# Mamba413/bess

Measured on AMD Instinct MI355X. Metric: candidate subsets solved/sec (n=50k,p=10k,k<=200 LM), higher is better.
Workload: dtype f64; 1 GPU; configs[1]: LM sequential path, Gaussian X n=50000 p=10000, s.list=1..200, GIC, warm start, max_iter=20, is_normal; score_pass=covariance updates (cached Gram columns), collective=none, ranks_with_work=1

## Files before the change

bess_amd/capi.py:

```python
import ctypes
import os
import sys

import numpy as np

_HERE = os.path.dirname(os.path.abspath(__file__))
LIB_PATH = os.environ.get("BESSX_LIB_PATH") or os.path.join(_HERE, "libbessx.so")

_D = ctypes.POINTER(ctypes.c_double)
_I = ctypes.POINTER(ctypes.c_int)
_i = ctypes.c_int
_d = ctypes.c_double
_ll = ctypes.c_longlong
_vp = ctypes.c_void_p

SYMBOLS = [
    "bessx_last_error", "bessx_device_info", "bessx_pywrap_bess", "bessx_bessCpp", "bessx_session_create",
    "bessx_session_destroy", "bessx_session_set_cv", "bessx_session_get_cv_folds", "bessx_session_sequential_path", "bessx_session_gs_path",
    "bessx_session_pgs_path", "bessx_session_get_screening", "bessx_session_get_screening_groups", "bessx_session_get_screening_scores", "bessx_session_score_mode", "bessx_session_counter",
    "bessx_session_trace_enable", "bessx_session_trace_size", "bessx_session_trace_copy_int",
    "bessx_session_trace_copy_double", "bessx_session_get_normalization", "bessx_session_score_pass_stats",
    "bessx_session_enable_kernel_timing", "bessx_session_submodel_steps", "bessx_session_fit", "bessx_session_fit_width", "bessx_session_reset_caches",
    "bessx_session_sequential_path_chain", "bessx_session_cv_eval", "bessx_session_debug_block_stream",
    "bessx_session_set_fill_hook", "bessx_session_set_kpath_chains",
# ... 575 lines not shown
        return int(lib().bessx_session_score_mode(self._h))

    def counters(self):
        names = {0: "chained_fits", 1: "cg_fallbacks", 2: "passes_over_X", 3: "chained_queued", 7: "cv_side_by_side_rounds",
                 8: "cv_union_fills", 9: "tie_rescues", 10: "cache_restarts", 11: "cv_contexts_dropped",
                 12: "cv_fold_contexts", 13: "shared_wide_fills", 14: "kpath_chunked_paths", 15: "kpath_stitch_refits",
                 16: "kpath_chunk_fills", 17: "kpath_chains_last_path",
                 18: "kpath_stitch_giveups", 19: "group_XTX_ns",
                 22: "kpath_coarse_us",
                 23: "kpath_chunks_us", 24: "kpath_stitch_us", 25: "panel_launches_one_group",
                 26: "panel_ns_one_group", 27: "panel_launches_two_groups", 28: "panel_ns_two_groups",
                 29: "shared_pass_launches", 30: "shared_pass_chain_slots", 31: "shared_pass_partial_batches",
                 32: "own_queue_streams_created_by_the_process", 33: "multi_responses_batched",
                 34: "multi_responses_host", 35: "multi_union_fills", 36: "x_bytes_uploaded_from_host",
                 37: "x_bytes_ingested_on_device", 38: "live_device_bytes_of_the_process",
                 39: "live_pinned_bytes_of_the_process", 40: "allocation_requests_of_the_process"}
        return {n: int(lib().bessx_session_counter(self._h, i)) for i, n in names.items()}

    def screening(self):
        a = np.zeros(self.p_kept, dtype=np.int32)
        lib().bessx_session_get_screening(self._h, _ip(a), a.size)
        return a

    def screening_groups(self):
        n = lib().bessx_session_get_screening_groups(self._h, None, 0)
        a = np.zeros(max(n, 1), dtype=np.int32)
        lib().bessx_session_get_screening_groups(self._h, _ip(a), n)
        return a[:n]

    def screening_scores(self):
        n = lib().bessx_session_get_screening_scores(self._h, None, 0)
# ... 1890 lines not shown
```

bess_amd/csrc/bessx_dev.h:

```cpp
#ifndef BESSX_DEV_H
#define BESSX_DEV_H

#include <hip/hip_runtime.h>

namespace bessx {

struct FitCtrl {
  int done;
  int l;
  int T0;
  int k_cur;
  int irls_done;
  int irls_steps;
  int info;
  int same_prev;
  double coef0;
  double ll0;
  int d_fresh;
  int irls_last;
  int fast_same;
  int ls_m;
  double ll1;
  int gram_full;
  int cov_nfill;
// ... 282 lines not shown
  int nblk, m;
  double *bcur, *bprev;
};
hipError_t launch_chol(const double *Gt, int m, int mt, double ridge, int ridge_skip0, const double *rhs,
                       const int *rhs_gather, double *sol, int *info, const FitCtrl *ctrl, int slot, int gate_mode,
                       hipStream_t st, const CholFuse *fuse = nullptr, const IrlsChk *chk = nullptr);
hipError_t launch_sym_fallback(const double *Gt, int m, int mt, double ridge, int ridge_skip0, const double *rhs,
                               const int *rhs_gather, double *sol, int *info, const FitCtrl *ctrl, int slot,
                               hipStream_t st, const CholFuse *fuse);
hipError_t launch_cg(int m, int mt, double ridge, const double *rhs, const int *A_new, double *sol, const FitCtrl *ctrl,
                     int slot, const CholFuse *fuse, int maxit, hipStream_t st, double tol = 1e-13, bool by_rows = true);
bool sel_cgr_applies(int len, int m);
hipError_t launch_sel_cgr(const double *score, int len, int k, int *A_new, const FitCtrl *ctrl, int slot,
                          const TopkNeed *need, double ridge, const double *rhs, double *sol, const CholFuse *fuse,
                          int maxit, hipStream_t st, double tol);
struct McState {
  int cand;
  int ncand;
  int need_d;
  int finished;
  int parked;
  int resume;
  int prev_fresh;
  int prev_T0;
  int solves;
  int why;
  int pad_[6];
};
static_assert(sizeof(McState) == 64, "McState is copied to the host in 64-byte records");
constexpr int MC_REC_I = 4;
// ... 218 lines not shown
```

bess_amd/csrc/bessx_fit.cpp:

```cpp
#include "bessx_host.h"

namespace bessx {

static int score_pass(bessx_session *s, int kind, int rs, int slot, std::vector<std::pair<size_t, bool>> &k1_pairs) {
  if (rs == 0 && shared_pass_applies(s)) {
    if (s->timing) k1_pairs.push_back({(size_t)-1, false});
    if (kind == 2 && s->cox.one_pass)
      return shared_pass_submit(s, nullptr, nullptr, s->part_rs[rs], nullptr, &s->cox, s->ctrl, slot);
    if (kind != 2)
      return shared_pass_submit(s, s->r_rs[rs], kind == 1 ? s->h_rs[rs] : nullptr, s->part_rs[rs],
                                kind == 1 ? s->part2_rs[rs] : nullptr, nullptr, s->ctrl, slot);
  }
  hipEvent_t ea = nullptr, eb = nullptr;
  if (int rc = k1_begin(s, &ea, &eb)) return rc;
  hipError_t e;
  if (kind == 2)
    e = launch_cox_score_pass(s->X, s->ld, s->p, s->U, s->nrb, s->cox, s->part_rs[rs], s->part2_rs[rs], s->ctrl, slot, s->st);
  else
    e = launch_xtv(s->X, s->ld, s->p, s->U, s->r_rs[rs], kind == 1 ? s->h_rs[rs] : nullptr, s->part_rs[rs],
                   kind == 1 ? s->part2_rs[rs] : nullptr, s->ctrl, slot, s->st);
  if (s->timing && e == hipSuccess) {
    e = hipEventRecord(eb, s->st);
    k1_pairs.push_back({s->ev_used - 2, false});
  }
// ... 122 lines not shown
    if (e != hipSuccess) return fail(BESSX_ERR_HIP, std::string("cov panel: ") + hipGetErrorString(e));
  }
  return 0;
}

int cov_C_dev(const bessx_session *s) { return s->cov_C - (s->cov_spec - COV_R); }

struct SlotFuse {
  const PubArgs *pub = nullptr;
  bool pub_fused = false;
  bool pub_snapshot = false;
  const PubArgs *attach = nullptr;
  bool attached = false;
  int cont_serial = 0, cont_parent = 0;
  bool cont = false, cont_fused = false;
};

CholFuse cov_fuse_args(bessx_session *s, int rs, int T0, bool force_chol, SlotFuse *sf) {
  bessx_session::CovCache &cv = s->cov[rs];
  CholFuse fz = {cv.G,          cv.slot_of, s->p,         T0,           s->ctrl,        s->A_cur, s->b_cur,
                 s->beta_dense, s->hist,    s->hist_beta, s->hist_coef0, s->hist_stride, s->inA,   s->yy_h[rs],
                 s->part_rs[rs], cv.GS, s->cov_cs,
                 cv.zero, PubArgs{}, s->fb_work, cv.meta + 4};
  if (sf && sf->pub && s->fuse && s->cov_cg && !force_chol && rs == 0) {
    fz.pub = *sf->pub;
    if (sf->pub_snapshot) fz.pub.on = 2;
    sf->pub_fused = true;
  }
  return fz;
}

// ... 83 lines not shown
    nd.cm_hist_coef0 = s->hist_coef0;
    nd.cm_hist_stride = s->hist_stride;
    nd.cm_inA = s->inA;
    nd.commit_on = (s->fuse && (T0 + 1 + 15) / 16 <= 16) ? 1 : 0;
    nd.no_restart = s->cov_no_restart ? 1 : 0;
    if (sf && sf->cont && s->fuse && slot == 1 && skip_d && scores_ok) {
      nd.cont_on = 1;
      nd.cont_serial = sf->cont_serial;
      nd.cont_parent = sf->cont_parent;
      sf->cont_fused = true;
      if (sf->attach) {
        nd.pub = *sf->attach;
        sf->attached = true;
      }
    }
    if (sf && sf->pub && sf->pub_snapshot && s->fuse && nd.commit_on && s->cov_cg && rs == 0) {
      nd.snap = *sf->pub;
      nd.snap.on = 2;
    }
    if (s->fuse_sel && s->fuse && s->cov_cg && s->cg_by_rows && sel_cgr_applies(s->p, T0)) {
      CholFuse fz = cov_fuse_args(s, rs, T0, false, sf);
      e = launch_sel_cgr(s->bd, s->p, T0, s->A_new, s->ctrl, slot, &nd, lambda, s->xty[rs], s->sol, &fz, 64, s->st,
                         s->cg_tol);
      if (e == hipSuccess && rs != 0)
        e = launch_resid_lm(s->X, s->ld, s->n, s->y, s->mask[rs], s->ctrl, slot, s->A_cur, s->b_cur, s->r_rs[rs],
                            s->sse, s->st, 1);
      if (e != hipSuccess) return fail(BESSX_ERR_HIP, std::string("enqueue_lm_slot_cov (fused): ") + hipGetErrorString(e));
      return 0;
    }
    e = launch_topk(s->bd, s->p, T0, s->A_new, s->cand, s->ctrl, slot, s->st, nullptr, &nd);
  } else if (e == hipSuccess) {
    e = launch_topk(s->bd, s->p, T0, s->A_new, s->cand, s->ctrl, slot, s->st, nullptr, nullptr, &s->tie);
    if (e == hipSuccess)
      e = launch_cov_need(s->A_new, T0, cov_speculates(s) ? s->bd : nullptr, s->bd2, s->p, cv.slot_of, cv.meta, cov_C_dev(s),
                          s->cov_fcols, s->ctrl, slot, s->A_cur, s->st, s->cov_no_restart ? 1 : 0);
  }
  if (e != hipSuccess) return fail(BESSX_ERR_HIP, std::string("enqueue_lm_slot_cov: ") + hipGetErrorString(e));
  return enqueue_cov_tail(s, slot, T0, lambda, rs, false, sf);
// ... 810 lines not shown
      s->trace.meta.push_back(s->n_train[rs]);
      s->trace.meta.push_back((int)s->trace.a_flat.size());
      for (size_t i = 0; i < cc.size(); i++) {
        s->trace.a_flat.push_back(cc[i]);
        s->trace.beta_flat.push_back(hb[(size_t)it * s->hist_stride + i]);
      }
      s->trace.coef0_calls.push_back(hc0[it]);
    }
  }
  return 0;
}

int enqueue_chained(bessx_session *s, const bessx_session::Hint &hint, int rs, int parent, int buf, int batch,
                           double parent_lambda, int parent_T0) {
  const int Tn = hint.T0;
  if (!(hint.on && s->chain && s->publish && s->warm_start && !s->trace.on && rs == 0 && s->cov_mode && Tn >= 1 &&
        Tn <= s->cap && Tn + COV_R + s->cov_spec <= s->cov_C && topk_supported(s->p, Tn)))
    return 0;
  bessx_session::Ahead &ah = s->ahead;
  s->chain_queued++;
  ah.armed = true;
  ah.T0 = Tn;
  ah.lambda = hint.lambda;
  ah.rs = rs;
  ah.serial = ++s->fit_serial;
  ah.buf = buf;
  const bool cont_fusable = s->fuse && hint.lambda == parent_lambda && topk_can_fuse_need(s->p);
  PubArgs parent_pub = {};
  const bool have_parent_pub = s->pend_on && cont_fusable && s->defer_pub;
  if (have_parent_pub) {
    parent_pub = s->pend;
    s->pend_on = false;
  } else if (int rc = publish_flush(s)) {
    return rc;
  }
  if (!cont_fusable) HIPX(launch_fit_continue(s->ctrl, Tn, s->hist, s->st, ah.serial, 1, parent));
  const PubArgs pa = publish_args(s, Tn, buf, &ah.seq);
  bool published = false, snapshotted = false;
  for (int b = 0, sl = 1; b < batch && sl <= s->max_iter; b++, sl++) {
    SlotFuse sf;
    const bool last = b + 1 == batch || sl == s->max_iter;
    if (last) {
      sf.pub = &pa;
      sf.pub_snapshot = s->defer_pub;
    }
    if (sl == 1 && cont_fusable) {
      sf.cont = true;
      sf.cont_serial = ah.serial;
      sf.cont_parent = parent;
      if (have_parent_pub) sf.attach = &parent_pub;
    }
    if (int rc = enqueue_lm_slot_cov(s, sl, Tn, hint.lambda, rs, sl == 1, hint.lambda == parent_lambda,
                                     hint.lambda == parent_lambda && Tn == parent_T0 + 1, &sf))
      return rc;
    if (sl == 1 && cont_fusable && !sf.cont_fused) return fail(BESSX_ERR_HIP, "internal: chained fit was not opened");
    if (sl == 1 && have_parent_pub && !sf.attached) return fail(BESSX_ERR_HIP, "internal: deferred publication lost");
    published = published || sf.pub_fused;
    snapshotted = snapshotted || (sf.pub_fused && sf.pub_snapshot);
  }
  if (snapshotted) {
    s->pend = publish_from_snapshot(pa);
    s->pend_on = true;
    return 0;
  }
  return published ? 0 : publish_launch(s, pa);
}


int algorithm_fit(bessx_session *s) {
  if (s->grouped) return algorithm_fit_grouped(s);
  const int T0 = s->sparsity_level, rs = s->cur_rows;
// ... 8 lines not shown
  if (!topk_supported(s->p, T0)) return fail(BESSX_ERR_UNSUPPORTED, "top-k selection: p too large for this sparsity level");
  const bool glm = s->model_type != 1;
  const bool cox = s->model_type == 4;
  const int k_init = (int)s->beta_init.idx.size();
  if (k_init > s->cap) return fail(BESSX_ERR_ARG, "initial support too large");
  bessx_session::RsCache &cc = s->cache[rs];
  const bool cov = s->cov_mode && !glm && T0 + COV_R + s->cov_spec <= s->cov_C && k_init + COV_R + s->cov_spec <= s->cov_C;
  bool use_cache = cc.valid && cc.coef0 == s->coef0_init && cc.beta.idx == s->beta_init.idx &&
                   cc.beta.val == s->beta_init.val && (!cox || s->cox_state_rs == rs) && (glm || cc.cov_layout == cov);
  if (cox) s->cox_state_rs = rs;
  bool model_kept = cov && !use_cache && cc.model_only && cc.cov_layout && s->dev_state_rs == rs &&
                          cc.coef0 == s->coef0_init && cc.beta.idx == s->beta_init.idx && cc.beta.val == s->beta_init.val &&
                          !s->trace.on && test_hook("model_kept") == nullptr;
  cc.valid = cc.model_only = false;
  const bessx_session::Hint hint = s->hint;
  s->hint.on = false;
  bool ahead_hit = false;
  int my_buf = 0, ahead_serial = 0;
  if (s->ahead.armed) {
    s->ahead.armed = false;
    const bessx_session::Ahead mine = s->ahead;
    if (cov && use_cache && s->dev_state_rs == rs && mine.T0 == T0 && mine.lambda == lambda && mine.rs == rs &&
        !s->trace.on) {
      if (int rc = enqueue_chained(s, hint, rs, mine.serial, mine.buf ^ 1, 2, lambda, T0)) return rc;
      if (!s->ahead.armed)
        if (int rc = publish_flush(s)) return rc;
      if (int rc = publish_wait(s, mine.buf, mine.seq)) return rc;
      ahead_hit = reinterpret_cast<const FitCtrl *>(s->res_h)->serial == mine.serial;
      if (!ahead_hit) {
        s->ahead.armed = false;
        s->pend_on = false;
      }
      (ahead_hit ? s->chain_hits : s->chain_dead)++;
      my_buf = mine.buf;
      ahead_serial = mine.serial;
    } else {
      HIPX(hipStreamSynchronize(s->st));
      s->pend_on = false;
      s->dev_state_rs = -1;
      use_cache = false;
      model_kept = false;
      s->chain_mismatch++;
    }
  }
  const int my_serial = ahead_hit ? ahead_serial : ++s->fit_serial;
  const bool scores_ok = cov && use_cache && s->dev_state_rs == rs && cc.cov_layout && cc.lambda == lambda;
  hipError_t e = hipSuccess;
  if (ahead_hit) {
  } else if ((use_cache && s->dev_state_rs == rs) || model_kept) {
    e = launch_fit_continue(s->ctrl, T0, s->hist, s->st, my_serial, 0);
  } else {
    int *st_idx = reinterpret_cast<int *>(s->stage_h);
    double *st_val = reinterpret_cast<double *>(s->stage_h + (size_t)s->capA * sizeof(int));
// ... 32 lines not shown
  }

  const FitCtrl *hc = reinterpret_cast<const FitCtrl *>(s->res_h);
  int slot = 1, batch = 2;
  std::vector<std::pair<size_t, bool>> k1_pairs;
  bool have_results = ahead_hit;
  if (ahead_hit) slot = 1 + std::min(batch, s->max_iter);
  while (!glm && cov) {
    if (!have_results) {
      const bool first_batch = slot == 1;
      unsigned long long seq = 0;
      PubArgs pa = {};
      if (s->publish) pa = publish_args(s, T0, my_buf, &seq);
      bool published = false;
      if (s->kch_owner && kchains_staged(s)) s->kch_gen_seen = kchains_generation(s);
      for (int b = 0; b < batch && slot <= s->max_iter; b++, slot++) {
        SlotFuse sf;
        if (s->publish && (b + 1 == batch || slot == s->max_iter)) sf.pub = &pa;
        if (int rc = enqueue_lm_slot_cov(s, slot, T0, lambda, rs, use_cache && slot == 1, scores_ok,
                                         scores_ok && cc.T0 + 1 == T0, &sf))
          return rc;
        published = published || sf.pub_fused;
      }
      if (!s->publish) {
        if (int rc = read_results(s, T0)) return rc;
      } else {
        if (!published)
          if (int rc = publish_launch(s, pa)) return rc;
        if (first_batch) {
          const auto tq = std::chrono::steady_clock::now();
          if (int rc = enqueue_chained(s, hint, rs, my_serial, my_buf ^ 1, batch, lambda, T0)) return rc;
          s->dbg_enq_s += std::chrono::duration<double>(std::chrono::steady_clock::now() - tq).count();
        }
        if (int rc = publish_wait(s, my_buf, seq)) return rc;
      }
    }
    have_results = false;
    hc = reinterpret_cast<const FitCtrl *>(s->res_h);
    if (int rc = cov_collect(s, hc->cov_nfill)) return rc;
    if (s->ahead.armed && !(hc->done && hc->d_fresh && !hc->info)) {
      s->ahead.armed = false;
      s->pend_on = false;
    }
    if (hc->cov_stall) {
      if (int rc = cov_unpark(s, hc, T0, lambda, rs, &slot)) return rc;
      continue;
    }
    if (hc->done || slot > s->max_iter) break;
  }
  const bool cgb_fit = cov && (T0 + 1 + 15) / 16 > 16 && s->cov_cg && T0 <= CGB_MAX_K && s->cgb_work != nullptr;
  if (cov && !hc->done && (rs != 0 || ((T0 + 1 + 15) / 16 > 16 && !cgb_fit) || !s->cov_cg)) {
    HIPX(launch_resid_lm(s->X, s->ld, s->n, s->y, s->mask[rs], s->ctrl, hc->l, s->A_cur, s->b_cur, s->r_rs[rs], s->sse,
                         s->st, 2));
    if (int rc = read_results(s, T0)) return rc;
    hc = reinterpret_cast<const FitCtrl *>(s->res_h);
  }
  if (cov) {
// ... 128 lines not shown
    }
  }
  s->sse_train = tr;
  s->sse_test = te;
  if (test_hook("fit_log"))
    std::fprintf(stderr, "[bessx] fit: level %d, %d iterations, started %s, scores kept %d, ended done=%d d_fresh=%d info=%d, slots queued %d\n", T0,
                 hc->l, ahead_hit ? "chained on the device" : (use_cache && s->dev_state_rs == rs ? "by k_fit_continue" : (model_kept ? "by k_fit_continue, scores formed again" : "from the host's copy")),
                 scores_ok ? 1 : 0, hc->done, hc->d_fresh, hc->info, slot - 1);
  cc.valid = hc->done && hc->d_fresh;
  cc.model_only = cov && hc->done && !hc->d_fresh && !hc->info && !hc->cov_miss;
  cc.cov_layout = cov;
  cc.lambda = lambda;
  cc.T0 = T0;
  cc.beta = s->beta;
  cc.coef0 = s->coef0;
  s->n_fits += 1;
  s->n_iters += hc->l;
  if (s->trace.on) {
    const int L = hc->l;
    std::vector<int> hh((size_t)(L + 1) * s->hist_stride);
    std::vector<double> hb((size_t)(L + 1) * s->hist_stride), hc0(L + 1);
    HIPX(hipMemcpy(hh.data(), s->hist, hh.size() * sizeof(int), hipMemcpyDeviceToHost));
    HIPX(hipMemcpy(hb.data(), s->hist_beta, hb.size() * sizeof(double), hipMemcpyDeviceToHost));
    HIPX(hipMemcpy(hc0.data(), s->hist_coef0, hc0.size() * sizeof(double), hipMemcpyDeviceToHost));
    for (int it = 1; it <= L; it++) {
      s->trace.meta.push_back(it);
      s->trace.meta.push_back(T0);
      s->trace.meta.push_back(s->n_train[rs]);
      s->trace.meta.push_back((int)s->trace.a_flat.size());
      for (int i = 0; i < T0; i++) {
// ... 13 lines not shown
```

bess_amd/csrc/bessx_host.h:

```cpp
#ifndef BESSX_HOST_H
#define BESSX_HOST_H
#include <hip/hip_runtime.h>

#include <algorithm>
#include <atomic>
#include <chrono>
#include <cfloat>
#include <cmath>
#include <cstdio>
#include <condition_variable>
#include <cstring>
#include <functional>
#include <mutex>
#include <numeric>
#include <random>
#include <string>
#include <thread>
#include <vector>

#include "../../include/bessx.h"
#include "bessx_dev.h"
#include "bessx_sync.h"

namespace bessx {
// ... 366 lines not shown
  FitCtrl *ctrl = nullptr;
  double *sse = nullptr, *b_cur = nullptr;
  int *A_cur = nullptr;
  int n_sse_blk = 0;
  unsigned char *res_h = nullptr;
  bool publish = true;
  unsigned long long *pub_flag = nullptr, pub_seq = 0;
  unsigned char *res_buf[2] = {nullptr, nullptr};
  unsigned char *snap[2] = {nullptr, nullptr};
  bool pend_on = false;
  PubArgs pend = {};
  struct Hint {
    bool on = false;
    int T0 = 0;
    double lambda = 0.0;
  } hint;
  struct Ahead {
    bool armed = false;
    int T0 = 0, rs = 0, serial = 0, buf = 0;
    double lambda = 0.0;
    unsigned long long seq = 0;
  } ahead;
  bool chain = true;
  long long chain_queued = 0, chain_hits = 0, chain_dead = 0, chain_mismatch = 0;
  int fit_serial = 0;
  unsigned char *stage_h = nullptr;
  std::vector<double> x_mean_h, x_norm_h;
  std::vector<int> cv_fold;
  std::vector<int> screen_groups, scr_gidx;
  std::vector<double> screen_scores;
  double y_mean_h = 0.0;
  double nullloss = 0.0;
  SparseVec beta;
  double coef0 = 0.0;
  SparseVec beta_init;
  double coef0_init = 0.0;
  int sparsity_level = 0;
  double lambda_level = 0.0;
  int cur_rows = 0;
// ... 176 lines not shown
```

bess_amd/csrc/bessx_k_solve.hip:

```cpp
#include "bessx_kdev.hpp"

namespace bessx {


__device__ __forceinline__ unsigned long long score_key(double v) {
  unsigned long long b = (unsigned long long)__double_as_longlong(v);
  return (b >> 63) ? 0ull : b;
}



template <int NT>
__device__ __forceinline__ bool repeated_set_body(const TopkNeed &nd, int k, int *__restrict__ out, int slot) {
  constexpr int NWV = NT / 64;
#ifdef BESSX_KTRACE
  unsigned long long tph_ = wall_clock64();
#endif
  PH(16);
  __shared__ double rmn[NWV], rmx[NWV];
  double mn = DBL_MAX, mx = -1.0;
  for (int b = threadIdx.x; b < nd.nbmm; b += NT) {
    mn = fmin(mn, nd.bmm[2 * b]);
    mx = fmax(mx, nd.bmm[2 * b + 1]);
  }
// ... 1527 lines not shown
  {
    asm volatile("s_waitcnt vmcnt(0) lgkmcnt(0)" ::: "memory");
    if (threadIdx.x == 0) {
      const unsigned long long kt3_ = wall_clock64();
      const int cls = ctrl->same_prev ? 0 : 1;
      atomicAdd(&g_phase[8 + 3 * cls], kt1_ - kt0_);
      atomicAdd(&g_phase[9 + 3 * cls], kt2_ - kt1_);
      atomicAdd(&g_phase[10 + 3 * cls], kt3_ - kt2_);
      atomicAdd(&g_phase[14 + cls], 1ull);
    }
  }
  KT(15);
#endif
}

template <int EB>
__device__ __noinline__ void mc_topk_call(const double *score, int p, int k, int *out, const FitCtrl *ctrl, int slot,
                                          const TopkNeed *nd) {
  topk_body<EB, 512>(score, nullptr, p, p, k, out, nullptr, ctrl, slot, nullptr, *nd);
}
template <int RPT, int NCW>
__device__ __noinline__ void mc_cgr_call(int m, int nc, double ridge, const double *rhs, const int *A_new, double *sol,
                                         const FitCtrl *ctrl, int slot, const CholFuse *fz, int maxit, double tol) {
  cgr_body<RPT, NCW>(m, nc, ridge, rhs, A_new, sol, ctrl, slot, *fz, maxit, tol);
}

template <int EB>
__global__ void __launch_bounds__(512) k_mc_sel_cgr(const McChain *__restrict__ chains) {
  const McChain &ch = chains[blockIdx.y];
  McState *st = ch.state;
// ... 525 lines not shown
    else                     \
      SC_GO(EB, 4, 26);      \
  } while (0)
  if (per <= 8)
    SC_BY_M(8);
  else if (per <= 24)
    SC_BY_M(24);
  else
    SC_BY_M(64);
#undef SC_BY_M
#undef SC_GO
  LAUNCH_CHECK();
  return hipSuccess;
}

bool mc_applies(int p, int kmax) { return sel_cgr_applies(p, kmax) && topk_can_fuse_need(p); }
hipError_t launch_mc_sel_cgr(const McChain *chains, int nchains, int p, hipStream_t st) {
  const int per = (p + 511) / 512;
  if (per <= 8)
    hipLaunchKernelGGL((k_mc_sel_cgr<8>), dim3(1, nchains), dim3(512), 0, st, chains);
  else if (per <= 24)
    hipLaunchKernelGGL((k_mc_sel_cgr<24>), dim3(1, nchains), dim3(512), 0, st, chains);
  else
    hipLaunchKernelGGL((k_mc_sel_cgr<64>), dim3(1, nchains), dim3(512), 0, st, chains);
  LAUNCH_CHECK();
  return hipSuccess;
}
hipError_t launch_mc_status(const McChain *chains, int nchains, unsigned char *host, unsigned long long *seq_host,
                            unsigned long long seq, hipStream_t st) {
  hipLaunchKernelGGL(k_mc_status, dim3(1), dim3(64), 0, st, chains, nchains, host, seq_host, seq);
// ... 48 lines not shown
```

bess_amd/csrc/bessx_kchunks.cpp:

```cpp
#include "bessx_host.h"
#include "bessx_kplan.h"
#include <optional>

namespace bessx {

struct SharedPass {
  PassRendezvous rdv;
  bool on = false;
  int kind = 0;
  int cap = XTV_MC_MAX;
  hipStream_t st = nullptr;
  std::mutex launch_mu;
  hipEvent_t ev_in[XTV_MC_MAX] = {};
  static constexpr int RING = 8;
  hipEvent_t ev_out[RING] = {};
  XtvMc xq = {};
  CoxMc cq = {};
  std::atomic<int> rc{0};
  void fail_with(hipError_t e) {
    int none = 0;
    if (e != hipSuccess) rc.compare_exchange_strong(none, (int)e);
  }
  bool timing = false;
  std::vector<hipEvent_t> tev;
// ... 1094 lines not shown
    s->beta.val.assign(q.last_val.begin(), q.last_val.begin() + q.last_len);
    s->coef0 = q.last_coef0;
  }
};

void fold_context_statistics(bessx_session *s, bessx_session *c) {
  auto take = [](auto &to, auto &from) { to += from, from = 0; };
  take(s->cov_panel_groups, c->cov_panel_groups);
  take(s->cov_cg_fallbacks, c->cov_cg_fallbacks);
  take(s->cov_tie_rescues, c->cov_tie_rescues);
  take(s->dbg_waits, c->dbg_waits);
  take(s->dbg_waits_ready, c->dbg_waits_ready);
  take(s->dbg_enq_s, c->dbg_enq_s);
  take(s->chain_queued, c->chain_queued);
  take(s->chain_hits, c->chain_hits);
  take(s->n_submodel_steps, c->n_submodel_steps);
  take(s->k1_seconds, c->k1_seconds);
  take(s->k1_bytes, c->k1_bytes);
  take(s->k1_launches, c->k1_launches);
  for (int w = 0; w < 2; w++) {
    take(s->panel_w_seconds[w], c->panel_w_seconds[w]);
    take(s->panel_w_launches[w], c->panel_w_launches[w]);
  }
}

}

int sequential_path_chunked(bessx_session *s, const int *seq, int ns, double lambda, int ic_type,
                            bessx_path_result *res, bessx_path_chain *link) {
  const int C = chains_for(s, ns, link != nullptr, link && link->init_len > 0 && link->keep_caches);
// ... 23 lines not shown
```

bess_amd/csrc/bessx_paths.cpp:

```cpp
#include "bessx_host.h"

namespace bessx {


void denormalize(const bessx_session *s, SparseVec &b, double &coef0, bool gs_variant) {
  if (!s->is_normal) return;
  double dot = 0.0, sn = std::sqrt((double)s->n);
  for (size_t i = 0; i < b.idx.size(); i++) {
    b.val[i] = sn * b.val[i] / s->x_norm_h[b.idx[i]];
    dot += b.val[i] * s->x_mean_h[b.idx[i]];
  }
  if (s->data_type == 1)
    coef0 = s->y_mean_h - dot;
  else if (s->data_type == 2 || gs_variant)
    coef0 = coef0 - dot;
}

int run_fit(bessx_session *s, int T0, double lambda, const SparseVec &beta_init, double coef0_init) {
  s->cur_rows = 0;
  s->sparsity_level = T0;
  s->lambda_level = lambda;
  s->beta_init = beta_init;
  s->coef0_init = coef0_init;
  return algorithm_fit(s);
// ... 63 lines not shown
      beta_init.idx.push_back(chain->init_idx[i]);
      beta_init.val.push_back(chain->init_val[i]);
    }
    coef0_init = chain->init_coef0;
    chain->stopped_at = -1;
    chain->last_len = 0;
    chain->last_coef0 = 0.0;
  }
  std::vector<Candidate> grid((size_t)ns * nl);
  std::vector<char> have((size_t)ns * nl, 0);
  bool stop = false;
  for (int i = 0; i < ns && !stop; i++) {
    int step = (i % 2 == 0) ? 1 : -1;
    for (int j = (i % 2 == 0) ? 0 : nl - 1; j < nl && j >= 0 && !stop; j += step) {
      {
        int jn = j + step, in = i;
        if (jn < 0 || jn >= nl) {
          in = i + 1;
          jn = (in % 2 == 0) ? 0 : nl - 1;
        }
        s->hint.on = in < ns && !is_cv;
        if (s->hint.on) {
          s->hint.T0 = seq[in];
          s->hint.lambda = lam[jn];
        }
      }
      if (int rc = run_fit(s, seq[i], lam[j], beta_init, coef0_init)) return rc;
      if (s->warm_start) {
        beta_init = s->beta;
        coef0_init = s->coef0;
      }
      Candidate &c = grid[(size_t)j * ns + i];
      have[(size_t)j * ns + i] = 1;
      c.T0 = seq[i];
      c.lambda = lam[j];
      c.beta = s->beta;
      c.coef0 = s->coef0;
      c.iters = s->l;
      if (int rc = metric_train_loss(s, &c.loss)) return rc;
// ... 424 lines not shown
}
#undef PW_TRY

struct PgsArgs {
  double lmin, lmax;
  int powell_path, nlambda;
};

int settle_device_chain(bessx_session *s) {
  kchains_quiesce(s);
  if (s->ahead.armed) {
    s->ahead.armed = false;
    HIPX(hipStreamSynchronize(s->st));
  }
  s->pend_on = false;
  s->hint.on = false;
  return 0;
}

int run_path(bessx_session *s, bool gs, const int *seq, int ns, const double *lam, int nl, int s_min,
                    int s_max, int ic_type, int is_cv, bessx_path_result *res, const PgsArgs *pgs,
                    bessx_path_chain *chain) {
  if (!s || !res) return fail(BESSX_ERR_ARG, "null session or result");
  if (is_cv && s->K < 2) return fail(BESSX_ERR_ARG, "is_cv needs bessx_session_set_cv first");
  HIPX(hipSetDevice(s->device));
  s->trace.clear();
  s->metric_depth = 0;
  for (auto &v : s->cv_init) v.clear();
  res->n_candidates = 0;
  s->n_fits = 0;
  s->n_iters = 0;
// ... 373 lines not shown
```

bess_amd/csrc/bessx_session.cpp:

```cpp
#include "bessx_host.h"

namespace bessx {

thread_local std::string g_err;
thread_local int g_marginal_fit_variant = 0;



void ctx_free(bessx_session *c) {
  if (!c) return;
  if (c->st) (void)hipStreamSynchronize(c->st);
  c->own.release();
  if (c->st) ctx_stream_destroy(c->st);
  delete c;
}

void drop_fold_contexts(bessx_session *s) {
  if (s->fold_pool) {
    s->fold_pool->stop();
    if (!s->fold_pool->broken) delete s->fold_pool;
    s->fold_pool = nullptr;
  }
  for (bessx_session *c : s->fold_ctx) ctx_free(c);
  s->fold_ctx.clear();
// ... 213 lines not shown
    if (std::chrono::duration<double>(std::chrono::steady_clock::now() - t0).count() > s->wait_deadline_s)
      return fail(BESSX_ERR_HIP, std::string(what) + ": the stream did not drain within " +
                                     std::to_string(s->wait_deadline_s) + " s (BESSX_WAIT_TIMEOUT_S) -- the session can "
                                     "only be destroyed now");
    if (spins > 2000) std::this_thread::sleep_for(std::chrono::microseconds(50));
  }
}

int reset_path_caches(bessx_session *s) {
  kchains_quiesce(s);
  if (s->ahead.armed) {
    s->ahead.armed = false;
    HIPX(hipStreamSynchronize(s->st));
  }
  s->pend_on = false;
  s->hint.on = false;
  for (auto &c : s->cache) c.valid = c.model_only = false;
  s->dev_state_rs = -1;
  for (bessx_session *c : s->fold_ctx) {
    HIPX(hipStreamSynchronize(c->st));
    for (auto &cc : c->cache) cc.valid = cc.model_only = false;
    c->dev_state_rs = -1;
  }
  for (auto &g : s->gcache) HIPX(hipMemsetAsync(g.meta, 0, 2 * sizeof(int), s->st));
  for (auto &c : s->cov) {
    HIPX(hipMemsetAsync(c.slot_of, 0xff, (size_t)s->p * sizeof(int), s->st));
    HIPX(hipMemsetAsync(c.meta, 0, 8 * sizeof(int), s->st));
  }
  return stream_wait_bounded(s, s->st, "clearing the path caches");
}

// ... 815 lines not shown
        s->cov_panel_blocks = (int)std::min<long>(panel_blocks, 1 << 30);
        s->cov_rps = (int)rps;
        s->cov_nslab = (int)ns;
        HIPT(s->own.alloc(&s->cov_part, (size_t)COV_SLOT_GROUPS * ns * njg * cov_streamed_tiles_per_wave() * 2 * 256));
        HIPT(s->own.alloc(&s->bd2, (size_t)p));
        HIPT(s->own.zeros(&s->inA, (size_t)p));
        HIPT(s->own.alloc(&s->cov_bmm, (size_t)3 * ((p + 31) / 32)));
        HIPT(s->own.alloc(&s->cov_fcols, (size_t)s->capA + 4 * COV_R));
        HIPT(s->own.alloc(&s->cov_extras, (size_t)2 * COV_R));
        TRY(alloc_cov_cache(s));
        HIPT(cov_panel_prepare());
        if (const char *ev = test_hook("cov_solver")) s->cov_cg = std::string(ev) != "chol";
        if (const char *ev = test_hook("fuse")) s->fuse = std::string(ev) != "0";
        if (const char *ev = test_hook("fuse_sel")) s->fuse_sel = std::string(ev) != "0";
        if (const char *ev = test_hook("defer_publish")) s->defer_pub = std::string(ev) != "0";
        if (!s->fuse) s->defer_pub = false;
        if (const char *ev = test_hook("cg_layout")) s->cg_by_rows = std::string(ev) != "tiles";
        if (const char *ev = test_hook("cov_cs")) s->cov_cs = std::min(COV_CS, std::max(1, std::atoi(ev)));
      } else if (mode == 2) {
        return bail(fail(BESSX_ERR_ARG, "covariance score mode: p too large for the Gram column cache"));
      }
    }
  }
  HIPT(s->own.alloc(&s->idcols, (size_t)capA + 16));
  if (s->model_type == 4) HIPT(cox_alloc(s));
  if (s->model_type == 1) {
    TRY(prepare_rowset(s, 0));
    if (const char *ev = test_hook("path_group_xtx")) s->path_group_xtx = std::string(ev) != "0";
  }
  HIPT(hipStreamSynchronize(s->st));
// ... 108 lines not shown
  bessx_session *c = new bessx_session(*ps);
  c->parent = ps;
  c->fold_pool = nullptr;
  c->fold_ctx.clear();
  c->ev_pool.clear();
  c->ev_used = 0;
  c->timing = false;
  c->trace = Trace();
  c->cov_timed.clear();
  c->publish = false;
  c->chain = false;
  c->defer_pub = false;
  c->cov_no_restart = true;
  c->hint = bessx_session::Hint();
  c->ahead = bessx_session::Ahead();
  c->pend_on = false;
  c->cache.assign(ps->cache.size(), bessx_session::RsCache());
  c->dev_state_rs = -1;
  c->bmm_owner = -1;
  c->fit_serial = 0;
  c->cur_rows = rs;
  c->n_fits = c->n_iters = 0;
  c->cov_cg_fallbacks = c->cov_tie_rescues = c->cov_panel_groups = 0;
  c->chain_queued = c->chain_hits = c->chain_dead = c->chain_mismatch = 0;
  c->dbg_waits = c->dbg_waits_ready = 0;
  c->pub_seq = 0;
  c->st = nullptr;
  const int p = ps->p, capA = ps->capA, mt_max = capA / 16;
  hipError_t e = hipSuccess;
  {
    const bool own_queue = own_queue_ok && ctx_stream_create(ps->device, &c->st);
    if (!own_queue) {
      int lo = 0, hi = 0;
      e = hipDeviceGetStreamPriorityRange(&lo, &hi);
      if (e == hipSuccess) e = hipStreamCreateWithPriority(&c->st, hipStreamNonBlocking, hi);
    }
    c->own_hw_queue = own_queue;
  }
  Owner &own = c->own;
// ... 421 lines not shown
    case 26: return (long long)(1e9 * s->panel_w_seconds[0]);
    case 27: return s->panel_w_launches[1];
    case 28: return (long long)(1e9 * s->panel_w_seconds[1]);
    case 29: return s->sp_launches;
    case 30: return s->sp_chain_slots;
    case 31: return s->sp_partial;
    case 32: return ctx_streams_created();
    case 33: return s->multi_batched;
    case 34: return s->multi_host;
    case 35: return s->multi_fills;
    case 36: return s->x_host_bytes;
    case 37: return s->x_dev_bytes;
    case 38: return Ledger::device_bytes.load();
    case 39: return Ledger::pinned_bytes.load();
    case 40: return Ledger::requests.load();
    case 10: {
      if (s->cov.empty()) return 0;
      int m[8] = {0, 0, 0, 0, 0, 0, 0, 0};
      if (hipSetDevice(s->device) != hipSuccess || hipStreamSynchronize(s->st) != hipSuccess ||
          hipMemcpy(m, s->cov[0].meta, sizeof(m), hipMemcpyDeviceToHost) != hipSuccess)
        return -1;
      return m[3];
    }
    default: return -1;
  }
}

int bessx_session_get_screening(const bessx_session *s, int *columns, int cap) {
  if (!s) return 0;
  for (int j = 0; j < s->p && j < cap && columns; j++) columns[j] = caller_col(s, j);
// ... 37 lines not shown
```

Before: 19250 candidates/s.

## Open the next chained fit's first slot inside the parent's select+CG launch

Adds a two-half fused kernel (k_sel_cgr2) that runs the parent fit's slot-2 top-k selection and CG solve, then immediately runs the first slot of the next path point's fit in the same launch. The path driver now passes a two-step-ahead hint, so the chained fit can adopt the already-opened slot and skip its own slot-1 launch. The goal is fewer kernel launches and less host enqueue work per candidate on the sequential LM path. In exchange it adds more host state (opened/stale tracking, invalidation when the hint does not match) and a single-block kernel doing double the serial work.

Result: no change. 19310 candidates/s (median of 2 runs) (+0.3%).

```diff
diff --git a/bess_amd/capi.py b/bess_amd/capi.py
--- a/bess_amd/capi.py
+++ b/bess_amd/capi.py
@@ -613,7 +613,8 @@
                  32: "own_queue_streams_created_by_the_process", 33: "multi_responses_batched",
                  34: "multi_responses_host", 35: "multi_union_fills", 36: "x_bytes_uploaded_from_host",
                  37: "x_bytes_ingested_on_device", 38: "live_device_bytes_of_the_process",
-                 39: "live_pinned_bytes_of_the_process", 40: "allocation_requests_of_the_process"}
+                 39: "live_pinned_bytes_of_the_process", 40: "allocation_requests_of_the_process",
+                 41: "chained_fits_opened_in_parent_launch"}
         return {n: int(lib().bessx_session_counter(self._h, i)) for i, n in names.items()}
 
     def screening(self):
diff --git a/bess_amd/csrc/bessx_dev.h b/bess_amd/csrc/bessx_dev.h
--- a/bess_amd/csrc/bessx_dev.h
+++ b/bess_amd/csrc/bessx_dev.h
@@ -320,6 +320,15 @@
 hipError_t launch_sel_cgr(const double *score, int len, int k, int *A_new, const FitCtrl *ctrl, int slot,
                           const TopkNeed *need, double ridge, const double *rhs, double *sol, const CholFuse *fuse,
                           int maxit, hipStream_t st, double tol);
+struct SelCgrHalf {
+  int k, slot, nc;
+  TopkNeed nd;
+  CholFuse fz;
+};
+bool sel_cgr_same_instance(int len, int k1, int k2);
+hipError_t launch_sel_cgr2(const double *score, int len, int *A_new, const FitCtrl *ctrl, const SelCgrHalf *a,
+                           const SelCgrHalf *b, double ridge, const double *rhs, double *sol, int maxit,
+                           hipStream_t st, double tol);
 struct McState {
   int cand;
   int ncand;
diff --git a/bess_amd/csrc/bessx_fit.cpp b/bess_amd/csrc/bessx_fit.cpp
--- a/bess_amd/csrc/bessx_fit.cpp
+++ b/bess_amd/csrc/bessx_fit.cpp
@@ -160,7 +160,21 @@
   bool attached = false;
   int cont_serial = 0, cont_parent = 0;
   bool cont = false, cont_fused = false;
+  bool attach_late = false;
+  bool next = false, next_fused = false;
+  int next_T0 = 0, next_serial = 0, next_parent = 0;
 };
+
+static bool chain_applies(const bessx_session *s, int Tn, int rs) {
+  return s->chain && s->publish && s->warm_start && !s->trace.on && rs == 0 && s->cov_mode && Tn >= 1 && Tn <= s->cap &&
+         Tn + COV_R + s->cov_spec <= s->cov_C && topk_supported(s->p, Tn);
+}
+
+static bool open_next_applies(const bessx_session *s, int rs, int T0, double lambda, bool on, int Tn, double lam_n) {
+  return on && s->fuse_next && s->fuse && s->fuse_sel && s->defer_pub && s->cov_cg && s->cg_by_rows && s->max_iter >= 2 &&
+         chain_applies(s, Tn, rs) && lam_n == lambda && topk_can_fuse_need(s->p) &&
+         sel_cgr_same_instance(s->p, T0, Tn) && (T0 + 1 + 15) / 16 <= 16 && (Tn + 1 + 15) / 16 <= 16;
+}
 
 CholFuse cov_fuse_args(bessx_session *s, int rs, int T0, bool force_chol, SlotFuse *sf) {
   bessx_session::CovCache &cv = s->cov[rs];
@@ -274,14 +288,38 @@
         sf->attached = true;
       }
     }
+    if (sf && sf->attach && sf->attach_late && s->fuse && !sf->attached) {
+      nd.pub = *sf->attach;
+      sf->attached = true;
+    }
     if (sf && sf->pub && sf->pub_snapshot && s->fuse && nd.commit_on && s->cov_cg && rs == 0) {
       nd.snap = *sf->pub;
       nd.snap.on = 2;
     }
     if (s->fuse_sel && s->fuse && s->cov_cg && s->cg_by_rows && sel_cgr_applies(s->p, T0)) {
       CholFuse fz = cov_fuse_args(s, rs, T0, false, sf);
-      e = launch_sel_cgr(s->bd, s->p, T0, s->A_new, s->ctrl, slot, &nd, lambda, s->xty[rs], s->sol, &fz, 64, s->st,
-                         s->cg_tol);
+      if (sf && sf->next && slot >= 2 && rs == 0 && sf->pub_fused && sel_cgr_same_instance(s->p, T0, sf->next_T0)) {
+        const int Tn = sf->next_T0;
+        SelCgrHalf ha = {T0, slot, (T0 + 7) / 8, nd, fz};
+        SelCgrHalf hb = ha;
+        hb.k = Tn;
+        hb.slot = 1;
+        hb.nc = (Tn + 7) / 8;
+        hb.nd.inc1 = Tn == T0 + 1 ? 1 : 0;
+        hb.nd.bmm_fresh = (Tn == T0 + 1 && s->bmm_owner == rs) ? 1 : 0;
+        hb.nd.snap = PubArgs{};
+        hb.nd.cont_on = 1;
+        hb.nd.cont_serial = sf->next_serial;
+        hb.nd.cont_parent = sf->next_parent;
+        hb.nd.commit_on = nd.commit_on;
+        hb.fz.T0 = Tn;
+        hb.fz.pub = PubArgs{};
+        e = launch_sel_cgr2(s->bd, s->p, s->A_new, s->ctrl, &ha, &hb, lambda, s->xty[rs], s->sol, 64, s->st, s->cg_tol);
+        sf->next_fused = e == hipSuccess;
+      } else {
+        e = launch_sel_cgr(s->bd, s->p, T0, s->A_new, s->ctrl, slot, &nd, lambda, s->xty[rs], s->sol, &fz, 64, s->st,
+                           s->cg_tol);
+      }
       if (e == hipSuccess && rs != 0)
         e = launch_resid_lm(s->X, s->ld, s->n, s->y, s->mask[rs], s->ctrl, slot, s->A_cur, s->b_cur, s->r_rs[rs],
                             s->sse, s->st, 1);
@@ -1122,17 +1160,24 @@
 int enqueue_chained(bessx_session *s, const bessx_session::Hint &hint, int rs, int parent, int buf, int batch,
                            double parent_lambda, int parent_T0) {
   const int Tn = hint.T0;
-  if (!(hint.on && s->chain && s->publish && s->warm_start && !s->trace.on && rs == 0 && s->cov_mode && Tn >= 1 &&
-        Tn <= s->cap && Tn + COV_R + s->cov_spec <= s->cov_C && topk_supported(s->p, Tn)))
+  const bessx_session::Opened op = s->opened;
+  s->opened.on = false;
+  const bool adopted = op.on && hint.on && op.T0 == Tn && op.lambda == hint.lambda && op.parent == parent &&
+                       hint.lambda == parent_lambda && batch >= 2 && chain_applies(s, Tn, rs);
+  if (op.on && !adopted) {
+    s->opened_stale = true;
     return 0;
+  }
+  if (!(hint.on && chain_applies(s, Tn, rs))) return 0;
   bessx_session::Ahead &ah = s->ahead;
   s->chain_queued++;
   ah.armed = true;
   ah.T0 = Tn;
   ah.lambda = hint.lambda;
   ah.rs = rs;
-  ah.serial = ++s->fit_serial;
+  ah.serial = adopted ? op.serial : ++s->fit_serial;
   ah.buf = buf;
+  ah.in_parent = adopted;
   const bool cont_fusable = s->fuse && hint.lambda == parent_lambda && topk_can_fuse_need(s->p);
   PubArgs parent_pub = {};
   const bool have_parent_pub = s->pend_on && cont_fusable && s->defer_pub;
@@ -1144,13 +1189,22 @@
   }
   if (!cont_fusable) HIPX(launch_fit_continue(s->ctrl, Tn, s->hist, s->st, ah.serial, 1, parent));
   const PubArgs pa = publish_args(s, Tn, buf, &ah.seq);
+  const bool open_next =
+      batch == 2 && cont_fusable && open_next_applies(s, rs, Tn, hint.lambda, hint.on2, hint.T0_2, hint.lambda2);
+  const int next_serial = open_next ? ++s->fit_serial : 0;
   bool published = false, snapshotted = false;
-  for (int b = 0, sl = 1; b < batch && sl <= s->max_iter; b++, sl++) {
+  for (int b = adopted ? 1 : 0, sl = adopted ? 2 : 1; b < batch && sl <= s->max_iter; b++, sl++) {
     SlotFuse sf;
     const bool last = b + 1 == batch || sl == s->max_iter;
     if (last) {
       sf.pub = &pa;
       sf.pub_snapshot = s->defer_pub;
+      if (open_next && sl == 2) {
+        sf.next = true;
+        sf.next_T0 = hint.T0_2;
+        sf.next_serial = next_serial;
+        sf.next_parent = ah.serial;
+      }
     }
     if (sl == 1 && cont_fusable) {
       sf.cont = true;
@@ -1158,11 +1212,23 @@
       sf.cont_parent = parent;
       if (have_parent_pub) sf.attach = &parent_pub;
     }
+    if (adopted && sl == 2 && have_parent_pub) {
+      sf.attach = &parent_pub;
+      sf.attach_late = true;
+    }
     if (int rc = enqueue_lm_slot_cov(s, sl, Tn, hint.lambda, rs, sl == 1, hint.lambda == parent_lambda,
                                      hint.lambda == parent_lambda && Tn == parent_T0 + 1, &sf))
       return rc;
     if (sl == 1 && cont_fusable && !sf.cont_fused) return fail(BESSX_ERR_HIP, "internal: chained fit was not opened");
-    if (sl == 1 && have_parent_pub && !sf.attached) return fail(BESSX_ERR_HIP, "internal: deferred publication lost");
+    if ((sl == 1 || (adopted && sl == 2)) && have_parent_pub && !sf.attached)
+      return fail(BESSX_ERR_HIP, "internal: deferred publication lost");
+    if (sf.next_fused) {
+      s->opened.on = true;
+      s->opened.T0 = hint.T0_2;
+      s->opened.lambda = hint.lambda2;
+      s->opened.serial = next_serial;
+      s->opened.parent = ah.serial;
+    }
     published = published || sf.pub_fused;
     snapshotted = snapshotted || (sf.pub_fused && sf.pub_snapshot);
   }
@@ -1201,7 +1267,7 @@
                           !s->trace.on && test_hook("model_kept") == nullptr;
   cc.valid = cc.model_only = false;
   const bessx_session::Hint hint = s->hint;
-  s->hint.on = false;
+  s->hint.on = s->hint.on2 = false;
   bool ahead_hit = false;
   int my_buf = 0, ahead_serial = 0;
   if (s->ahead.armed) {
@@ -1217,13 +1283,16 @@
       if (!ahead_hit) {
         s->ahead.armed = false;
         s->pend_on = false;
+        s->opened.on = s->opened_stale = false;
       }
       (ahead_hit ? s->chain_hits : s->chain_dead)++;
+      if (ahead_hit && mine.in_parent) s->chain_in_parent++;
       my_buf = mine.buf;
       ahead_serial = mine.serial;
     } else {
       HIPX(hipStreamSynchronize(s->st));
       s->pend_on = false;
+      s->opened.on = s->opened_stale = false;
       s->dev_state_rs = -1;
       use_cache = false;
       model_kept = false;
@@ -1286,12 +1355,28 @@
       if (s->publish) pa = publish_args(s, T0, my_buf, &seq);
       bool published = false;
       if (s->kch_owner && kchains_staged(s)) s->kch_gen_seen = kchains_generation(s);
+      const bool open_next = first_batch && batch == 2 && s->publish &&
+                             open_next_applies(s, rs, T0, lambda, hint.on, hint.T0, hint.lambda);
+      const int next_serial = open_next ? ++s->fit_serial : 0;
       for (int b = 0; b < batch && slot <= s->max_iter; b++, slot++) {
         SlotFuse sf;
         if (s->publish && (b + 1 == batch || slot == s->max_iter)) sf.pub = &pa;
+        if (open_next && sf.pub && slot == 2) {
+          sf.next = true;
+          sf.next_T0 = hint.T0;
+          sf.next_serial = next_serial;
+          sf.next_parent = my_serial;
+        }
         if (int rc = enqueue_lm_slot_cov(s, slot, T0, lambda, rs, use_cache && slot == 1, scores_ok,
                                          scores_ok && cc.T0 + 1 == T0, &sf))
           return rc;
+        if (sf.next_fused) {
+          s->opened.on = true;
+          s->opened.T0 = hint.T0;
+          s->opened.lambda = hint.lambda;
+          s->opened.serial = next_serial;
+          s->opened.parent = my_serial;
+        }
         published = published || sf.pub_fused;
       }
       if (!s->publish) {
@@ -1313,6 +1398,7 @@
     if (s->ahead.armed && !(hc->done && hc->d_fresh && !hc->info)) {
       s->ahead.armed = false;
       s->pend_on = false;
+      s->opened.on = false;
     }
     if (hc->cov_stall) {
       if (int rc = cov_unpark(s, hc, T0, lambda, rs, &slot)) return rc;
@@ -1471,6 +1557,11 @@
   cc.T0 = T0;
   cc.beta = s->beta;
   cc.coef0 = s->coef0;
+  if (s->opened_stale) {
+    s->opened_stale = false;
+    cc.valid = cc.model_only = false;
+    s->dev_state_rs = -1;
+  }
   s->n_fits += 1;
   s->n_iters += hc->l;
   if (s->trace.on) {
diff --git a/bess_amd/csrc/bessx_host.h b/bess_amd/csrc/bessx_host.h
--- a/bess_amd/csrc/bessx_host.h
+++ b/bess_amd/csrc/bessx_host.h
@@ -404,15 +404,27 @@
     bool on = false;
     int T0 = 0;
     double lambda = 0.0;
+    bool on2 = false;
+    int T0_2 = 0;
+    double lambda2 = 0.0;
   } hint;
   struct Ahead {
     bool armed = false;
     int T0 = 0, rs = 0, serial = 0, buf = 0;
     double lambda = 0.0;
     unsigned long long seq = 0;
+    bool in_parent = false;
   } ahead;
+  struct Opened {
+    bool on = false;
+    int T0 = 0, serial = 0, parent = 0;
+    double lambda = 0.0;
+  } opened;
+  bool opened_stale = false;
   bool chain = true;
+  bool fuse_next = true;
   long long chain_queued = 0, chain_hits = 0, chain_dead = 0, chain_mismatch = 0;
+  long long chain_in_parent = 0;
   int fit_serial = 0;
   unsigned char *stage_h = nullptr;
   std::vector<double> x_mean_h, x_norm_h;
diff --git a/bess_amd/csrc/bessx_k_solve.hip b/bess_amd/csrc/bessx_k_solve.hip
--- a/bess_amd/csrc/bessx_k_solve.hip
+++ b/bess_amd/csrc/bessx_k_solve.hip
@@ -1565,6 +1565,40 @@
 #endif
 }
 
+template <int EB, int RPT, int NCW>
+__global__ void __launch_bounds__(512) k_sel_cgr2(const double *__restrict__ score, int len, int *out,
+                                                  const FitCtrl *ctrl, const SelCgrHalf ha, const SelCgrHalf hb,
+                                                  double ridge, const double *__restrict__ rhs, double *sol, int maxit,
+                                                  const double tol) {
+  KT(14);
+  if (ha.nd.pub.on && blockIdx.x == 1) {
+    publish_body(ha.nd.pub);
+    return;
+  }
+  bool settled = false;
+  if (!ha.nd.cont_on && ha.nd.commit_on && ha.nd.slot_of != nullptr && !ctrl->done && ctrl->l == ha.slot - 1 &&
+      ctrl->l >= 1 && ha.nd.ctrl->fast_same)
+    settled = repeated_set_body<512>(ha.nd, ha.k, out, ha.slot);
+  if (!settled) {
+    topk_body<EB, 512>(score, nullptr, len, len, ha.k, out, nullptr, ctrl, ha.slot, nullptr, ha.nd);
+    __syncthreads();
+    cgr_body<RPT, NCW>(ha.k, ha.nc, ridge, rhs, out, sol, ctrl, ha.slot, ha.fz, maxit, tol);
+  }
+  if (ha.fz.pub.on) {
+    __syncthreads();
+    if (ha.fz.pub.on == 2) {
+      if (ha.fz.ctrl->snap_seq != ha.fz.pub.seq) snapshot_body(ha.fz.pub);
+    } else {
+      publish_body(ha.fz.pub);
+    }
+  }
+  __syncthreads();
+  topk_body<EB, 512>(score, nullptr, len, len, hb.k, out, nullptr, ctrl, hb.slot, nullptr, hb.nd);
+  __syncthreads();
+  cgr_body<RPT, NCW>(hb.k, hb.nc, ridge, rhs, out, sol, ctrl, hb.slot, hb.fz, maxit, tol);
+  KT(15);
+}
+
 template <int EB>
 __device__ __noinline__ void mc_topk_call(const double *score, int p, int k, int *out, const FitCtrl *ctrl, int slot,
                                           const TopkNeed *nd) {
@@ -2120,6 +2154,44 @@
   return hipSuccess;
 }
 
+static int sel_cgr_bucket(int k) { return k <= 64 ? 0 : (k <= 128 ? 1 : (k <= 192 ? 2 : 3)); }
+bool sel_cgr_same_instance(int len, int k1, int k2) {
+  return sel_cgr_applies(len, k1) && sel_cgr_applies(len, k2) && sel_cgr_bucket(k1) == sel_cgr_bucket(k2);
+}
+hipError_t launch_sel_cgr2(const double *score, int len, int *A_new, const FitCtrl *ctrl, const SelCgrHalf *a,
+                           const SelCgrHalf *b, double ridge, const double *rhs, double *sol, int maxit,
+                           hipStream_t st, double tol) {
+  if (a == nullptr || b == nullptr || !sel_cgr_same_instance(len, a->k, b->k) || b->nd.pub.on != a->nd.pub.on ||
+      b->fz.pub.on || b->nd.snap.on || !b->nd.cont_on)
+    return hipErrorInvalidValue;
+  const SelCgrHalf ha = *a, hb = *b;
+  const int nblk = ha.nd.pub.on ? 2 : 1, per = (len + 511) / 512, k = ha.k;
+#define SC_GO(EB, RP, NW_)                                                                                          \
+  hipLaunchKernelGGL((k_sel_cgr2<EB, RP, NW_>), dim3(nblk), dim3(512), 0, st, score, len, A_new, ctrl, ha, hb, ridge, \
+                     rhs, sol, maxit, tol)
+#define SC_BY_M(EB)          \
+  do {                       \
+    if (k <= 64)             \
+      SC_GO(EB, 1, 8);       \
+    else if (k <= 128)       \
+      SC_GO(EB, 2, 16);      \
+    else if (k <= 192)       \
+      SC_GO(EB, 3, 24);      \
+    else                     \
+      SC_GO(EB, 4, 26);      \
+  } while (0)
+  if (per <= 8)
+    SC_BY_M(8);
+  else if (per <= 24)
+    SC_BY_M(24);
+  else
+    SC_BY_M(64);
+#undef SC_BY_M
+#undef SC_GO
+  LAUNCH_CHECK();
+  return hipSuccess;
+}
+
 bool mc_applies(int p, int kmax) { return sel_cgr_applies(p, kmax) && topk_can_fuse_need(p); }
 hipError_t launch_mc_sel_cgr(const McChain *chains, int nchains, int p, hipStream_t st) {
   const int per = (p + 511) / 512;
diff --git a/bess_amd/csrc/bessx_kchunks.cpp b/bess_amd/csrc/bessx_kchunks.cpp
--- a/bess_amd/csrc/bessx_kchunks.cpp
+++ b/bess_amd/csrc/bessx_kchunks.cpp
@@ -1132,6 +1132,7 @@
   take(s->dbg_enq_s, c->dbg_enq_s);
   take(s->chain_queued, c->chain_queued);
   take(s->chain_hits, c->chain_hits);
+  take(s->chain_in_parent, c->chain_in_parent);
   take(s->n_submodel_steps, c->n_submodel_steps);
   take(s->k1_seconds, c->k1_seconds);
   take(s->k1_bytes, c->k1_bytes);
diff --git a/bess_amd/csrc/bessx_paths.cpp b/bess_amd/csrc/bessx_paths.cpp
--- a/bess_amd/csrc/bessx_paths.cpp
+++ b/bess_amd/csrc/bessx_paths.cpp
@@ -101,15 +101,26 @@
     int step = (i % 2 == 0) ? 1 : -1;
     for (int j = (i % 2 == 0) ? 0 : nl - 1; j < nl && j >= 0 && !stop; j += step) {
       {
-        int jn = j + step, in = i;
-        if (jn < 0 || jn >= nl) {
-          in = i + 1;
-          jn = (in % 2 == 0) ? 0 : nl - 1;
-        }
+        auto after = [&](int &in, int &jn) {
+          jn += (in % 2 == 0) ? 1 : -1;
+          if (jn < 0 || jn >= nl) {
+            in = in + 1;
+            jn = (in % 2 == 0) ? 0 : nl - 1;
+          }
+        };
+        int in = i, jn = j;
+        after(in, jn);
         s->hint.on = in < ns && !is_cv;
+        s->hint.on2 = false;
         if (s->hint.on) {
           s->hint.T0 = seq[in];
           s->hint.lambda = lam[jn];
+          after(in, jn);
+          s->hint.on2 = in < ns;
+          if (s->hint.on2) {
+            s->hint.T0_2 = seq[in];
+            s->hint.lambda2 = lam[jn];
+          }
         }
       }
       if (int rc = run_fit(s, seq[i], lam[j], beta_init, coef0_init)) return rc;
@@ -564,7 +575,8 @@
     HIPX(hipStreamSynchronize(s->st));
   }
   s->pend_on = false;
-  s->hint.on = false;
+  s->opened.on = false;
+  s->hint.on = s->hint.on2 = false;
   return 0;
 }
 
diff --git a/bess_amd/csrc/bessx_session.cpp b/bess_amd/csrc/bessx_session.cpp
--- a/bess_amd/csrc/bessx_session.cpp
+++ b/bess_amd/csrc/bessx_session.cpp
@@ -251,7 +251,8 @@
     HIPX(hipStreamSynchronize(s->st));
   }
   s->pend_on = false;
-  s->hint.on = false;
+  s->opened.on = s->opened_stale = false;
+  s->hint.on = s->hint.on2 = false;
   for (auto &c : s->cache) c.valid = c.model_only = false;
   s->dev_state_rs = -1;
   for (bessx_session *c : s->fold_ctx) {
@@ -1097,6 +1098,7 @@
         if (const char *ev = test_hook("fuse")) s->fuse = std::string(ev) != "0";
         if (const char *ev = test_hook("fuse_sel")) s->fuse_sel = std::string(ev) != "0";
         if (const char *ev = test_hook("defer_publish")) s->defer_pub = std::string(ev) != "0";
+        if (const char *ev = test_hook("fuse_next")) s->fuse_next = std::string(ev) != "0";
         if (!s->fuse) s->defer_pub = false;
         if (const char *ev = test_hook("cg_layout")) s->cg_by_rows = std::string(ev) != "tiles";
         if (const char *ev = test_hook("cov_cs")) s->cov_cs = std::min(COV_CS, std::max(1, std::atoi(ev)));
@@ -1235,6 +1237,8 @@
   c->cov_no_restart = true;
   c->hint = bessx_session::Hint();
   c->ahead = bessx_session::Ahead();
+  c->opened = bessx_session::Opened();
+  c->opened_stale = false;
   c->pend_on = false;
   c->cache.assign(ps->cache.size(), bessx_session::RsCache());
   c->dev_state_rs = -1;
@@ -1243,7 +1247,7 @@
   c->cur_rows = rs;
   c->n_fits = c->n_iters = 0;
   c->cov_cg_fallbacks = c->cov_tie_rescues = c->cov_panel_groups = 0;
-  c->chain_queued = c->chain_hits = c->chain_dead = c->chain_mismatch = 0;
+  c->chain_queued = c->chain_hits = c->chain_dead = c->chain_mismatch = c->chain_in_parent = 0;
   c->dbg_waits = c->dbg_waits_ready = 0;
   c->pub_seq = 0;
   c->st = nullptr;
@@ -1695,6 +1699,7 @@
     case 38: return Ledger::device_bytes.load();
     case 39: return Ledger::pinned_bytes.load();
     case 40: return Ledger::requests.load();
+    case 41: return s->chain_in_parent;
     case 10: {
       if (s->cov.empty()) return 0;
       int m[8] = {0, 0, 0, 0, 0, 0, 0, 0};
```
